# MCG-NJU/LinK

Measured on AMD Instinct MI355X. Metric: voxels/s through one LinK (3x7)^3 block, 100k active voxels C=64, higher is better.
Workload: dtype f32

## Files before the change

link_amd/csrc/dense_batch.hip:

```cpp
#define DC_IO 0
#define DC_IO_NS dcb_f32
#include "dense_batch_impl.h"

namespace dcb_f16 { int batch_set_launch(const link::dc_bt_host_t &, const link_dc_buffers_t *, const int64_t *, int, const link_dc_grid_t &, const link_elk_desc_t &); }
namespace dcb_bf16 { int batch_set_launch(const link::dc_bt_host_t &, const link_dc_buffers_t *, const int64_t *, int, const link_dc_grid_t &, const link_elk_desc_t &); }

using namespace link;
using namespace dcb_f32;

static constexpr int BT_RING = 4;
__global__ void k_dc_batch_spin(unsigned long long *stamp, int ticks) {
  const unsigned long long t0 = __builtin_amdgcn_s_memrealtime();
  if (threadIdx.x == 0) *stamp = t0;
  while (__builtin_amdgcn_s_memrealtime() - t0 < (unsigned long long)ticks) __builtin_amdgcn_s_sleep(16);
}
static bool bt_queue_delay_us(hipStream_t x, hipStream_t y, unsigned long long *scratch , hipEvent_t ev, double *us) {
  unsigned long long h[2] = {0, 0};
  *us = 0.0;
  if (hipStreamSynchronize(x) != hipSuccess || hipStreamSynchronize(y) != hipSuccess) return false;
  hipLaunchKernelGGL(k_dc_batch_spin, dim3(1), dim3(64), 0, x, scratch, 15000);
  if (hipEventRecord(ev, x) != hipSuccess) return false;
  hipLaunchKernelGGL(k_dc_batch_spin, dim3(1), dim3(64), 0, y, scratch + 1, 0);
  if (hipStreamSynchronize(x) != hipSuccess || hipStreamSynchronize(y) != hipSuccess ||
      hipMemcpy(h, scratch, sizeof h, hipMemcpyDeviceToHost) != hipSuccess)
    return false;
  *us = ((double)h[1] - (double)h[0]) / 100.0;
  return true;
}
static bool bt_share_queue(hipStream_t x, hipStream_t y, unsigned long long *scratch, hipEvent_t ev) {
  double d = 0.0;
  return !bt_queue_delay_us(x, y, scratch, ev, &d) || d > 75.0;
}
struct link_dc_batch {
  int device, cus;
  hipStream_t sa, sb, sc;
  std::vector<hipStream_t> pool;
  int ia, ib;
  std::vector<std::pair<hipStream_t, unsigned>> callers;
  unsigned long long *probe_scratch;
  hipEvent_t probe_ev;
  bool timing;
  hipEvent_t tb[BT_RING][3], te[BT_RING][3];
  bool timed[BT_RING];
  int32_t *sync;
  hipEvent_t ev_in[BT_RING], ev_ms[BT_RING], ev_a[BT_RING], ev_c[BT_RING], ev_out[BT_RING];
  std::vector<const void *> bufs[BT_RING];
  bool used[BT_RING];
  long long calls;
  unsigned long long *dbg1, *dbg2;
};

extern "C" int link_dc_batch_create(link_dc_batch_t **out) {
  if (!out) return LINK_ERR_ARG;
  link_dc_batch *c = new link_dc_batch();
  hipDeviceProp_t pr;
  if (hipGetDevice(&c->device) != hipSuccess || hipGetDeviceProperties(&pr, c->device) != hipSuccess) { delete c; return LINK_ERR_LAUNCH; }
  c->cus = pr.multiProcessorCount;
  int pr_lo = 0, pr_hi = 0;
  (void)hipDeviceGetStreamPriorityRange(&pr_lo, &pr_hi);
  bool ok = hipStreamCreateWithPriority(&c->sc, hipStreamNonBlocking, pr_hi) == hipSuccess &&
            hipMalloc(reinterpret_cast<void **>(&c->probe_scratch), 16) == hipSuccess &&
            hipEventCreateWithFlags(&c->probe_ev, hipEventDisableTiming) == hipSuccess;
  std::vector<hipStream_t> rejected;
  const bool dbg_place = getenv("LINK_DC_BATCH_DEBUG") != nullptr;
  for (int cand = 0; ok && cand < 12 && c->pool.size() < 4; cand++) {
    hipStream_t s_ = nullptr;
    if (hipStreamCreateWithFlags(&s_, hipStreamNonBlocking) != hipSuccess) { ok = false; break; }
    bool bad = bt_share_queue(c->sc, s_, c->probe_scratch, c->probe_ev);
    for (size_t i = 0; i < c->pool.size() && !bad; i++) bad = bt_share_queue(c->pool[i], s_, c->probe_scratch, c->probe_ev);
    (bad ? rejected : c->pool).push_back(s_);
  }
  while (ok && c->pool.size() < 2 && !rejected.empty()) { c->pool.push_back(rejected.back()); rejected.pop_back(); }
  for (hipStream_t s_ : rejected) (void)hipStreamDestroy(s_);
  ok = ok && c->pool.size() >= 2;
  if (ok) { c->ia = 0; c->ib = 1; c->sa = c->pool[0]; c->sb = c->pool[1]; }
  if (dbg_place)
    fprintf(stderr, "link_dc_batch_create: %zu streams on hardware queues of their own, %zu candidates rejected\n",
            c->pool.size(), rejected.size());
  ok = ok && hipMalloc(reinterpret_cast<void **>(&c->sync), sizeof(int32_t) * BT_RING * BT_SYNC_WORDS) == hipSuccess &&
            hipMemset(c->sync, 0, sizeof(int32_t) * BT_RING * BT_SYNC_WORDS) == hipSuccess;
  for (int i = 0; i < BT_RING && ok; i++) {
#ifndef DC_BT_EVENT_FLAGS
#define DC_BT_EVENT_FLAGS (hipEventDisableTiming | hipEventDisableSystemFence)
#endif
    ok = hipEventCreateWithFlags(&c->ev_in[i], DC_BT_EVENT_FLAGS) == hipSuccess && hipEventCreateWithFlags(&c->ev_ms[i], DC_BT_EVENT_FLAGS) == hipSuccess &&
         hipEventCreateWithFlags(&c->ev_a[i], DC_BT_EVENT_FLAGS) == hipSuccess && hipEventCreateWithFlags(&c->ev_c[i], DC_BT_EVENT_FLAGS) == hipSuccess &&
         hipEventCreateWithFlags(&c->ev_out[i], DC_BT_EVENT_FLAGS) == hipSuccess;
    c->used[i] = false;
  }
  c->calls = 0;
  c->dbg1 = c->dbg2 = nullptr;
  if (!ok) { (void)hipGetLastError(); delete c; return LINK_ERR_LAUNCH; }
  *out = c;
  return LINK_OK;
}

extern "C" int link_dc_batch_destroy(link_dc_batch_t *c) {
  if (!c) return LINK_OK;
  (void)hipStreamSynchronize(c->sa); (void)hipStreamSynchronize(c->sb); (void)hipStreamSynchronize(c->sc);
  for (int i = 0; i < BT_RING; i++) {
    (void)hipEventDestroy(c->ev_in[i]); (void)hipEventDestroy(c->ev_ms[i]); (void)hipEventDestroy(c->ev_a[i]); (void)hipEventDestroy(c->ev_c[i]);
    (void)hipEventDestroy(c->ev_out[i]);
  }
  for (int i = 0; i < BT_RING; i++)
    for (int k = 0; k < 3; k++) { if (c->tb[i][k]) (void)hipEventDestroy(c->tb[i][k]); if (c->te[i][k]) (void)hipEventDestroy(c->te[i][k]); }
  (void)hipFree(c->sync);
  (void)hipFree(c->probe_scratch);
  (void)hipEventDestroy(c->probe_ev);
  for (hipStream_t s_ : c->pool) (void)hipStreamDestroy(s_);
  (void)hipStreamDestroy(c->sc);
  delete c;
  return LINK_OK;
}

extern "C" int link_dc_batch_set_debug(link_dc_batch_t *c, uint64_t *k1_rows, uint64_t *k2_rows) {
  if (!c) return LINK_ERR_ARG;
  c->dbg1 = reinterpret_cast<unsigned long long *>(k1_rows);
  c->dbg2 = reinterpret_cast<unsigned long long *>(k2_rows);
  return DC_BT_PROF ? LINK_OK : 1;
}

extern "C" int link_streams_share_queue(void *a, void *b, double *delay_us) {
  if (!delay_us) return LINK_ERR_ARG;
  unsigned long long *st = nullptr;
  hipEvent_t ev;
  if (hipMalloc(reinterpret_cast<void **>(&st), 16) != hipSuccess) return LINK_ERR_LAUNCH;
  if (hipEventCreateWithFlags(&ev, hipEventDisableTiming) != hipSuccess) { (void)hipFree(st); return LINK_ERR_LAUNCH; }
  const bool ok = bt_queue_delay_us(S(a), S(b), st, ev, delay_us);
  (void)hipEventDestroy(ev);
  (void)hipFree(st);
  if (!ok) { (void)hipGetLastError(); return LINK_ERR_LAUNCH; }
  return LINK_OK;
}

extern "C" int link_dc_batch_probe_streams(link_dc_batch_t *c, hipStream_t caller, double *delays_us ) {
  if (!c || !delays_us) return LINK_ERR_ARG;
  unsigned long long *st = nullptr;
  hipEvent_t ev;
  if (hipMalloc(reinterpret_cast<void **>(&st), 16) != hipSuccess) return LINK_ERR_LAUNCH;
  if (hipEventCreateWithFlags(&ev, hipEventDisableTiming) != hipSuccess) { (void)hipFree(st); return LINK_ERR_LAUNCH; }
  hipStream_t xs[12] = {c->sa, c->sa, c->sb, caller, caller, caller, c->sb, c->sc, c->sc, c->sa, c->sb, c->sc},
              ys[12] = {c->sb, c->sc, c->sc, c->sa, c->sb, c->sc, c->sa, c->sa, c->sb, caller, caller, caller};
  bool ok = true;
  for (int i = 0; i < 12; i++) ok = bt_queue_delay_us(xs[i], ys[i], st, ev, &delays_us[i]) && ok;
  (void)hipEventDestroy(ev);
  (void)hipFree(st);
  if (!ok) { (void)hipGetLastError(); return LINK_ERR_LAUNCH; }
  return LINK_OK;
}

extern "C" int link_dc_batch_set_timing(link_dc_batch_t *c, int32_t on) {
  if (!c) return LINK_ERR_ARG;
  c->timing = on != 0;
  return LINK_OK;
}
extern "C" int link_dc_batch_kernel_times(link_dc_batch_t *c, int64_t ticket, float *ms ) {
  if (!c || !ms || ticket < 0 || ticket >= c->calls || c->calls - ticket > BT_RING) return LINK_ERR_ARG;
  const int q = (int)(ticket % BT_RING);
  if (!c->timed[q]) return LINK_ERR_ARG;
  for (int i = 0; i < 3; i++)
    if (hipEventSynchronize(c->te[q][i]) != hipSuccess || hipEventElapsedTime(&ms[i], c->tb[q][i], c->te[q][i]) != hipSuccess) {
      (void)hipGetLastError();
      return LINK_ERR_LAUNCH;
    }
  return LINK_OK;
}

extern "C" int link_dc_batch_status(link_dc_batch_t *c, int32_t *out) {
  if (!c || !out) return LINK_ERR_ARG;
  if (hipStreamSynchronize(c->sa) != hipSuccess || hipStreamSynchronize(c->sb) != hipSuccess || hipStreamSynchronize(c->sc) != hipSuccess)
    return LINK_ERR_LAUNCH;
  out[0] = 0;
  out[1] = (int32_t)c->calls;
  for (int i = 0; i < BT_RING; i++) {
    int32_t e = 0;
    if (hipMemcpy(&e, c->sync + (size_t)i * BT_SYNC_WORDS + bt_err(), sizeof(e), hipMemcpyDeviceToHost) != hipSuccess) return LINK_ERR_LAUNCH;
    if (e && !out[0]) out[0] = e;
  }
  return out[0] ? LINK_BATCH_TIMEOUT : LINK_OK;
}

__global__ void k_dc_batch_clear(int32_t *sync, int words) {
  for (int i = threadIdx.x; i < words; i += blockDim.x) sync[i] = 0;
}

static void bt_mind_caller(link_dc_batch *c, hipStream_t st) {
  unsigned mask = 0;
  bool known = false;
  for (auto &e : c->callers) if (e.first == st) { mask = e.second; known = true; break; }
  if (!known) {
    hipStreamCaptureStatus cap = hipStreamCaptureStatusNone;
    if (hipStreamIsCapturing(st, &cap) != hipSuccess || cap != hipStreamCaptureStatusNone) {
      (void)hipGetLastError();
      return;
    }
    for (size_t i = 0; i < c->pool.size(); i++)
      if (bt_share_queue(st, c->pool[i], c->probe_scratch, c->probe_ev)) mask |= 1u << i;
    if (c->callers.size() >= 16) c->callers.erase(c->callers.begin());
    c->callers.emplace_back(st, mask);
    if (getenv("LINK_DC_BATCH_DEBUG")) fprintf(stderr, "link_dc_batch: caller stream %p shares a hardware queue with pool streams mask 0x%x\n", (void *)st, mask);
  }
  if (!(mask & (1u << c->ia)) && !(mask & (1u << c->ib))) return;
  int na = -1, nb = -1;
  for (int i = 0; i < (int)c->pool.size(); i++)
    if (!(mask & (1u << i))) { if (na < 0) na = i; else if (nb < 0) nb = i; }
  if (na < 0 || nb < 0) return;
  (void)hipStreamSynchronize(c->sa); (void)hipStreamSynchronize(c->sb); (void)hipStreamSynchronize(c->sc);
  c->ia = na; c->ib = nb; c->sa = c->pool[na]; c->sb = c->pool[nb];
}

extern "C" int link_dc_batch_submit(link_dc_batch_t *c, const link_dc_buffers_t *frames, const int64_t *n, int32_t nframes,
                                    const link_dc_grid_t *g, const link_elk_desc_t *d, void *stream, int64_t *ticket) {
  if (ticket) *ticket = -1;
  if (!c || !g || !d || nframes < 0 || (nframes > 0 && (!frames || !n))) return LINK_ERR_ARG;
  if (nframes == 0) return LINK_OK;
  if (d->c != 64 || d->cg != 32 || (d->op != LINK_OP_COS && d->op != LINK_OP_SIN) || (d->r != 2 && d->r != 3) || d->coord_div != 1.0f) return LINK_ERR_ARG;
  if (g->k < DC_INL || g->k > 352 || g->vp * (int64_t)g->k * 16 >= (1LL << 32) || (g->vp + 1) * (int64_t)2 * 64 * 4 >= (1LL << 32)) return LINK_ERR_ARG;
  if constexpr (!(dc_k2q_cfg<LINK_OP_COS, 3>::FITS && dc_k2q_cfg<LINK_OP_COS, 2>::FITS)) return LINK_ERR_ARG;
  const link_dc_buffers_t &b0 = frames[0];
  for (int i = 0; i < nframes; i++) {
    const link_dc_buffers_t &b = frames[i];
    if (n[i] <= 0 || n[i] >= (1LL << 29) || n[i] * 64 * 4 >= (1LL << 32) || b.io_dtype != b0.io_dtype || b.alpha) return LINK_ERR_ARG;
    if (!b.feats || !b.coords || !b.slots || !b.cnt || !b.cell_n || !b.vcell || !b.S || !b.hdr || !b.out) return LINK_ERR_ARG;
    if (b.w_pre != b0.w_pre || b.pre_ln_w != b0.pre_ln_w || b.pre_ln_b != b0.pre_ln_b || b.w_pos != b0.w_pos || b.ln_w != b0.ln_w || b.ln_b != b0.ln_b)
      return LINK_ERR_ARG;
    for (int k = 0; k < i; k++)
      if (frames[k].S == b.S || frames[k].cnt == b.cnt || frames[k].out == b.out) return LINK_ERR_ARG;
  }
  if (!b0.w_pre || !b0.pre_ln_w || !b0.pre_ln_b || !b0.w_pos || !b0.ln_w || !b0.ln_b) return LINK_ERR_ARG;
  int dev = -1;
  if (hipGetDevice(&dev) != hipSuccess || dev != c->device) return LINK_ERR_ARG;
  hipStream_t st = S(stream);
  bt_mind_caller(c, st);
  for (int base = 0; base < nframes; base += DC_BT_MAX) {
    const int nb = nframes - base < DC_BT_MAX ? nframes - base : DC_BT_MAX;
    const int q = (int)(c->calls % BT_RING);
    std::vector<const void *> keys;
    for (int i = 0; i < nb; i++) keys.push_back(frames[base + i].S);
    bool fail = hipEventRecord(c->ev_in[q], st) != hipSuccess;
    fail = fail || hipStreamWaitEvent(c->sa, c->ev_in[q], 0) != hipSuccess || hipStreamWaitEvent(c->sb, c->ev_in[q], 0) != hipSuccess ||
           hipStreamWaitEvent(c->sc, c->ev_in[q], 0) != hipSuccess;
    for (int r = 0; r < BT_RING && !fail; r++) {
      if (!c->used[r]) continue;
      bool dep = r == q;
      for (size_t i = 0; i < keys.size() && !dep; i++)
        for (size_t k = 0; k < c->bufs[r].size() && !dep; k++) dep = keys[i] == c->bufs[r][k];
      if (dep)
        fail = hipStreamWaitEvent(c->sa, c->ev_out[r], 0) != hipSuccess || hipStreamWaitEvent(c->sc, c->ev_out[r], 0) != hipSuccess ||
               hipStreamWaitEvent(c->sa, c->ev_a[r], 0) != hipSuccess || hipStreamWaitEvent(c->sc, c->ev_a[r], 0) != hipSuccess;
    }
    int32_t *sync = c->sync + (size_t)q * BT_SYNC_WORDS;
#ifndef DC_BT_CLEAR_ON_INSERT
#define DC_BT_CLEAR_ON_INSERT 1
#endif
    hipStream_t s_clear = DC_BT_CLEAR_ON_INSERT ? c->sc : c->sa, s_o1 = DC_BT_CLEAR_ON_INSERT ? c->sa : c->sc;
    if (!fail) hipLaunchKernelGGL(k_dc_batch_clear, dim3(1), dim3(256), 0, s_clear, sync, (int)BT_SYNC_WORDS);
    fail = fail || hipEventRecord(c->ev_ms[q], s_clear) != hipSuccess ||
           hipStreamWaitEvent(c->sb, c->ev_ms[q], 0) != hipSuccess || hipStreamWaitEvent(s_o1, c->ev_ms[q], 0) != hipSuccess;
    if (fail) { (void)hipGetLastError(); return LINK_ERR_LAUNCH; }
    int rc;
    hipStream_t role3[3] = {c->sc, c->sa, c->sb};
    c->timed[q] = false;
    if (c->timing) {
      bool okt = true;
      for (int i = 0; i < 3 && okt; i++) {
        if (!c->tb[q][i]) okt = hipEventCreate(&c->tb[q][i]) == hipSuccess && hipEventCreate(&c->te[q][i]) == hipSuccess;
        okt = okt && hipEventRecord(c->tb[q][i], role3[i]) == hipSuccess;
      }
      c->timed[q] = okt;
    }
    const dc_bt_host_t hset{c->sa, c->sb, c->sc, c->cus, sync, c->dbg1, c->dbg2};
    if (b0.io_dtype == LINK_IO_F16) rc = dcb_f16::batch_set_launch(hset, frames + base, n + base, nb, *g, *d);
    else if (b0.io_dtype == LINK_IO_BF16) rc = dcb_bf16::batch_set_launch(hset, frames + base, n + base, nb, *g, *d);
    else rc = dcb_f32::batch_set_launch(hset, frames + base, n + base, nb, *g, *d);
    if (c->timed[q])
      for (int i = 0; i < 3; i++) c->timed[q] = hipEventRecord(c->te[q][i], role3[i]) == hipSuccess && c->timed[q];
    fail = hipEventRecord(c->ev_a[q], c->sa) != hipSuccess || hipEventRecord(c->ev_c[q], c->sc) != hipSuccess || hipEventRecord(c->ev_out[q], c->sb) != hipSuccess;
    c->bufs[q] = keys;
    c->used[q] = true;
    if (ticket) *ticket = c->calls;
    c->calls++;
    if (rc != LINK_OK || fail) {
      (void)hipStreamWaitEvent(st, c->ev_a[q], 0); (void)hipStreamWaitEvent(st, c->ev_c[q], 0); (void)hipStreamWaitEvent(st, c->ev_out[q], 0);
      if (rc != LINK_OK) return rc;
      (void)hipGetLastError();
      return LINK_ERR_LAUNCH;
    }
  }
  return LINK_OK;
}

extern "C" int link_dc_batch_join(link_dc_batch_t *c, int64_t ticket, void *stream) {
  if (!c || ticket < 0 || ticket >= c->calls) return LINK_ERR_ARG;
  const int q = (int)(ticket % BT_RING);
  hipStream_t st = S(stream);
  if (hipStreamWaitEvent(st, c->ev_a[q], 0) != hipSuccess || hipStreamWaitEvent(st, c->ev_c[q], 0) != hipSuccess ||
      hipStreamWaitEvent(st, c->ev_out[q], 0) != hipSuccess) {
    (void)hipGetLastError();
    return LINK_ERR_LAUNCH;
  }
  return LINK_OK;
}

extern "C" int link_elk_core_dense_forward_batch(link_dc_batch_t *c, const link_dc_buffers_t *frames, const int64_t *n, int32_t nframes,
                                                 const link_dc_grid_t *g, const link_elk_desc_t *d, void *stream) {
  int64_t ticket = -1;
  const int rc = link_dc_batch_submit(c, frames, n, nframes, g, d, stream, &ticket);
  if (rc != LINK_OK || ticket < 0) return rc;
  return link_dc_batch_join(c, ticket, stream);
}
```

Before: 3.381 billion.

## Optionally alternate pre_mix kernels across two pool streams and slim insert waits

Adds an optional mode, off by default, that alternates the pre_mix kernel stream between two hardware-queue pool streams on even and odd launch sets, so consecutive sets can overlap. It also changes the submit path unconditionally. The input event and buffer-dependency waits now go only to the clear stream, not to all three role streams, relying on the clear kernel's event to order the others. Join waits on the previous set's pre_mix event when the streams differ, which adds some cross-set dependency bookkeeping.

```diff
diff --git a/link_amd/csrc/dense_batch.hip b/link_amd/csrc/dense_batch.hip
--- a/link_amd/csrc/dense_batch.hip
+++ b/link_amd/csrc/dense_batch.hip
@@ -34,8 +34,11 @@
 struct link_dc_batch {
   int device, cus;
   hipStream_t sa, sb, sc;
+  hipStream_t sa2;
   std::vector<hipStream_t> pool;
-  int ia, ib;
+  int ia, ib, ia2;
+  bool alt_want;
+  hipStream_t k1s[BT_RING];
   std::vector<std::pair<hipStream_t, unsigned>> callers;
   unsigned long long *probe_scratch;
   hipEvent_t probe_ev;
@@ -49,6 +52,24 @@
   long long calls;
   unsigned long long *dbg1, *dbg2;
 };
+
+#ifndef DC_BT_ALTERNATE_DEFAULT
+#define DC_BT_ALTERNATE_DEFAULT 0
+#endif
+static bool bt_sync_all(link_dc_batch *c) {
+  bool ok = true;
+  for (hipStream_t s_ : c->pool) ok = hipStreamSynchronize(s_) == hipSuccess && ok;
+  return hipStreamSynchronize(c->sc) == hipSuccess && ok;
+}
+static void bt_say_mode(const link_dc_batch *c, const char *when) {
+  if (!getenv("LINK_DC_BATCH_DEBUG")) return;
+  if (c->sa2)
+    fprintf(stderr, "link_dc_batch (%s): pre_mix kernels ALTERNATE between pool streams %d (even launch sets) and %d (odd), gather on %d\n", when, c->ia,
+            c->ia2, c->ib);
+  else
+    fprintf(stderr, "link_dc_batch (%s): every pre_mix kernel on pool stream %d, gather on %d (%s)\n", when, c->ia, c->ib,
+            c->alt_want ? "no third pool stream on a hardware queue of its own" : "alternation switched off");
+}
 
 extern "C" int link_dc_batch_create(link_dc_batch_t **out) {
   if (!out) return LINK_ERR_ARG;
@@ -73,10 +94,17 @@
   while (ok && c->pool.size() < 2 && !rejected.empty()) { c->pool.push_back(rejected.back()); rejected.pop_back(); }
   for (hipStream_t s_ : rejected) (void)hipStreamDestroy(s_);
   ok = ok && c->pool.size() >= 2;
-  if (ok) { c->ia = 0; c->ib = 1; c->sa = c->pool[0]; c->sb = c->pool[1]; }
+  const char *alt_env = getenv("LINK_DC_BATCH_ALTERNATE");
+  c->alt_want = alt_env ? atoi(alt_env) != 0 : DC_BT_ALTERNATE_DEFAULT != 0;
+  c->sa2 = nullptr; c->ia2 = -1;
+  if (ok) {
+    c->ia = 0; c->ib = 1; c->sa = c->pool[0]; c->sb = c->pool[1];
+    if (c->alt_want && c->pool.size() >= 3) { c->ia2 = 2; c->sa2 = c->pool[2]; }
+  }
   if (dbg_place)
     fprintf(stderr, "link_dc_batch_create: %zu streams on hardware queues of their own, %zu candidates rejected\n",
             c->pool.size(), rejected.size());
+  if (ok) bt_say_mode(c, "create");
   ok = ok && hipMalloc(reinterpret_cast<void **>(&c->sync), sizeof(int32_t) * BT_RING * BT_SYNC_WORDS) == hipSuccess &&
             hipMemset(c->sync, 0, sizeof(int32_t) * BT_RING * BT_SYNC_WORDS) == hipSuccess;
   for (int i = 0; i < BT_RING && ok; i++) {
@@ -87,6 +115,7 @@
          hipEventCreateWithFlags(&c->ev_a[i], DC_BT_EVENT_FLAGS) == hipSuccess && hipEventCreateWithFlags(&c->ev_c[i], DC_BT_EVENT_FLAGS) == hipSuccess &&
          hipEventCreateWithFlags(&c->ev_out[i], DC_BT_EVENT_FLAGS) == hipSuccess;
     c->used[i] = false;
+    c->k1s[i] = nullptr;
   }
   c->calls = 0;
   c->dbg1 = c->dbg2 = nullptr;
@@ -97,7 +126,7 @@
 
 extern "C" int link_dc_batch_destroy(link_dc_batch_t *c) {
   if (!c) return LINK_OK;
-  (void)hipStreamSynchronize(c->sa); (void)hipStreamSynchronize(c->sb); (void)hipStreamSynchronize(c->sc);
+  (void)bt_sync_all(c);
   for (int i = 0; i < BT_RING; i++) {
     (void)hipEventDestroy(c->ev_in[i]); (void)hipEventDestroy(c->ev_ms[i]); (void)hipEventDestroy(c->ev_a[i]); (void)hipEventDestroy(c->ev_c[i]);
     (void)hipEventDestroy(c->ev_out[i]);
@@ -143,6 +172,12 @@
               ys[12] = {c->sb, c->sc, c->sc, c->sa, c->sb, c->sc, c->sa, c->sa, c->sb, caller, caller, caller};
   bool ok = true;
   for (int i = 0; i < 12; i++) ok = bt_queue_delay_us(xs[i], ys[i], st, ev, &delays_us[i]) && ok;
+  for (int i = 0; i < 12 && c->sa2; i++) {
+    if (xs[i] != c->sa && ys[i] != c->sa) continue;
+    double d2 = 0.0;
+    ok = bt_queue_delay_us(xs[i] == c->sa ? c->sa2 : xs[i], ys[i] == c->sa ? c->sa2 : ys[i], st, ev, &d2) && ok;
+    if (d2 > delays_us[i]) delays_us[i] = d2;
+  }
   (void)hipEventDestroy(ev);
   (void)hipFree(st);
   if (!ok) { (void)hipGetLastError(); return LINK_ERR_LAUNCH; }
@@ -168,8 +203,7 @@
 
 extern "C" int link_dc_batch_status(link_dc_batch_t *c, int32_t *out) {
   if (!c || !out) return LINK_ERR_ARG;
-  if (hipStreamSynchronize(c->sa) != hipSuccess || hipStreamSynchronize(c->sb) != hipSuccess || hipStreamSynchronize(c->sc) != hipSuccess)
-    return LINK_ERR_LAUNCH;
+  if (!bt_sync_all(c)) return LINK_ERR_LAUNCH;
   out[0] = 0;
   out[1] = (int32_t)c->calls;
   for (int i = 0; i < BT_RING; i++) {
@@ -200,13 +234,25 @@
     c->callers.emplace_back(st, mask);
     if (getenv("LINK_DC_BATCH_DEBUG")) fprintf(stderr, "link_dc_batch: caller stream %p shares a hardware queue with pool streams mask 0x%x\n", (void *)st, mask);
   }
-  if (!(mask & (1u << c->ia)) && !(mask & (1u << c->ib))) return;
-  int na = -1, nb = -1;
+  if (!(mask & (1u << c->ia)) && !(mask & (1u << c->ib)) && !(c->ia2 >= 0 && (mask & (1u << c->ia2)))) return;
+  int na = -1, nb = -1, na2 = -1;
   for (int i = 0; i < (int)c->pool.size(); i++)
-    if (!(mask & (1u << i))) { if (na < 0) na = i; else if (nb < 0) nb = i; }
+    if (!(mask & (1u << i))) { if (na < 0) na = i; else if (nb < 0) nb = i; else if (na2 < 0) na2 = i; }
   if (na < 0 || nb < 0) return;
-  (void)hipStreamSynchronize(c->sa); (void)hipStreamSynchronize(c->sb); (void)hipStreamSynchronize(c->sc);
+  (void)bt_sync_all(c);
   c->ia = na; c->ib = nb; c->sa = c->pool[na]; c->sb = c->pool[nb];
+  c->ia2 = c->alt_want ? na2 : -1;
+  c->sa2 = c->ia2 >= 0 ? c->pool[c->ia2] : nullptr;
+  bt_say_mode(c, "roles moved off the caller's queue");
+}
+
+static bool bt_join_set(link_dc_batch *c, long long ticket, hipStream_t st) {
+  const int q = (int)(ticket % BT_RING), q1 = (int)((ticket + BT_RING - 1) % BT_RING);
+  bool ok = hipStreamWaitEvent(st, c->ev_a[q], 0) == hipSuccess;
+  ok = hipStreamWaitEvent(st, c->ev_c[q], 0) == hipSuccess && ok;
+  ok = hipStreamWaitEvent(st, c->ev_out[q], 0) == hipSuccess && ok;
+  if (ticket >= 1 && c->used[q1] && c->k1s[q1] != c->k1s[q]) ok = hipStreamWaitEvent(st, c->ev_a[q1], 0) == hipSuccess && ok;
+  return ok;
 }
 
 extern "C" int link_dc_batch_submit(link_dc_batch_t *c, const link_dc_buffers_t *frames, const int64_t *n, int32_t nframes,
@@ -237,29 +283,34 @@
     const int q = (int)(c->calls % BT_RING);
     std::vector<const void *> keys;
     for (int i = 0; i < nb; i++) keys.push_back(frames[base + i].S);
+    hipStream_t sk = (c->sa2 && (c->calls & 1)) ? c->sa2 : c->sa;
+#ifndef DC_BT_CLEAR_ON_INSERT
+#define DC_BT_CLEAR_ON_INSERT 1
+#endif
+    hipStream_t s_clear = DC_BT_CLEAR_ON_INSERT ? c->sc : sk, s_o1 = DC_BT_CLEAR_ON_INSERT ? sk : c->sc;
     bool fail = hipEventRecord(c->ev_in[q], st) != hipSuccess;
-    fail = fail || hipStreamWaitEvent(c->sa, c->ev_in[q], 0) != hipSuccess || hipStreamWaitEvent(c->sb, c->ev_in[q], 0) != hipSuccess ||
-           hipStreamWaitEvent(c->sc, c->ev_in[q], 0) != hipSuccess;
+    fail = fail || hipStreamWaitEvent(s_clear, c->ev_in[q], 0) != hipSuccess;
     for (int r = 0; r < BT_RING && !fail; r++) {
       if (!c->used[r]) continue;
       bool dep = r == q;
       for (size_t i = 0; i < keys.size() && !dep; i++)
         for (size_t k = 0; k < c->bufs[r].size() && !dep; k++) dep = keys[i] == c->bufs[r][k];
-      if (dep)
-        fail = hipStreamWaitEvent(c->sa, c->ev_out[r], 0) != hipSuccess || hipStreamWaitEvent(c->sc, c->ev_out[r], 0) != hipSuccess ||
-               hipStreamWaitEvent(c->sa, c->ev_a[r], 0) != hipSuccess || hipStreamWaitEvent(c->sc, c->ev_a[r], 0) != hipSuccess;
-    }
+      if (dep) fail = hipStreamWaitEvent(s_clear, c->ev_out[r], 0) != hipSuccess || hipStreamWaitEvent(s_clear, c->ev_a[r], 0) != hipSuccess;
+    }
+    const int q3 = (int)((c->calls + 1) % BT_RING);
+    if (!fail && c->sa2 && c->calls >= 3 && c->used[q3]) fail = hipStreamWaitEvent(s_clear, c->ev_a[q3], 0) != hipSuccess;
     int32_t *sync = c->sync + (size_t)q * BT_SYNC_WORDS;
-#ifndef DC_BT_CLEAR_ON_INSERT
-#define DC_BT_CLEAR_ON_INSERT 1
-#endif
-    hipStream_t s_clear = DC_BT_CLEAR_ON_INSERT ? c->sc : c->sa, s_o1 = DC_BT_CLEAR_ON_INSERT ? c->sa : c->sc;
     if (!fail) hipLaunchKernelGGL(k_dc_batch_clear, dim3(1), dim3(256), 0, s_clear, sync, (int)BT_SYNC_WORDS);
     fail = fail || hipEventRecord(c->ev_ms[q], s_clear) != hipSuccess ||
            hipStreamWaitEvent(c->sb, c->ev_ms[q], 0) != hipSuccess || hipStreamWaitEvent(s_o1, c->ev_ms[q], 0) != hipSuccess;
-    if (fail) { (void)hipGetLastError(); return LINK_ERR_LAUNCH; }
+    if (fail) {
+      (void)hipGetLastError();
+      if (base > 0) (void)bt_join_set(c, c->calls - 1, st);
+      (void)hipGetLastError();
+      return LINK_ERR_LAUNCH;
+    }
     int rc;
-    hipStream_t role3[3] = {c->sc, c->sa, c->sb};
+    hipStream_t role3[3] = {c->sc, sk, c->sb};
     c->timed[q] = false;
     if (c->timing) {
       bool okt = true;
@@ -269,19 +320,20 @@
       }
       c->timed[q] = okt;
     }
-    const dc_bt_host_t hset{c->sa, c->sb, c->sc, c->cus, sync, c->dbg1, c->dbg2};
+    const dc_bt_host_t hset{sk, c->sb, c->sc, c->cus, sync, c->dbg1, c->dbg2};
     if (b0.io_dtype == LINK_IO_F16) rc = dcb_f16::batch_set_launch(hset, frames + base, n + base, nb, *g, *d);
     else if (b0.io_dtype == LINK_IO_BF16) rc = dcb_bf16::batch_set_launch(hset, frames + base, n + base, nb, *g, *d);
     else rc = dcb_f32::batch_set_launch(hset, frames + base, n + base, nb, *g, *d);
     if (c->timed[q])
       for (int i = 0; i < 3; i++) c->timed[q] = hipEventRecord(c->te[q][i], role3[i]) == hipSuccess && c->timed[q];
-    fail = hipEventRecord(c->ev_a[q], c->sa) != hipSuccess || hipEventRecord(c->ev_c[q], c->sc) != hipSuccess || hipEventRecord(c->ev_out[q], c->sb) != hipSuccess;
+    fail = hipEventRecord(c->ev_a[q], sk) != hipSuccess || hipEventRecord(c->ev_c[q], c->sc) != hipSuccess || hipEventRecord(c->ev_out[q], c->sb) != hipSuccess;
     c->bufs[q] = keys;
     c->used[q] = true;
+    c->k1s[q] = sk;
     if (ticket) *ticket = c->calls;
     c->calls++;
     if (rc != LINK_OK || fail) {
-      (void)hipStreamWaitEvent(st, c->ev_a[q], 0); (void)hipStreamWaitEvent(st, c->ev_c[q], 0); (void)hipStreamWaitEvent(st, c->ev_out[q], 0);
+      (void)bt_join_set(c, c->calls - 1, st);
       if (rc != LINK_OK) return rc;
       (void)hipGetLastError();
       return LINK_ERR_LAUNCH;
@@ -292,10 +344,7 @@
 
 extern "C" int link_dc_batch_join(link_dc_batch_t *c, int64_t ticket, void *stream) {
   if (!c || ticket < 0 || ticket >= c->calls) return LINK_ERR_ARG;
-  const int q = (int)(ticket % BT_RING);
-  hipStream_t st = S(stream);
-  if (hipStreamWaitEvent(st, c->ev_a[q], 0) != hipSuccess || hipStreamWaitEvent(st, c->ev_c[q], 0) != hipSuccess ||
-      hipStreamWaitEvent(st, c->ev_out[q], 0) != hipSuccess) {
+  if (!bt_join_set(c, ticket, S(stream))) {
     (void)hipGetLastError();
     return LINK_ERR_LAUNCH;
   }
```

Result: no change. 3.366 billion (-0.4%).
